# rvp-group/srrg2_proslam

Hardware: AMD Instinct MI355X
Metric: tracked frames/sec on KITTI-00 stereo (1241x376, ~2k kp); SE(3) vs ref (higher is better)
Workload: dtype u64 popcount (Hamming) + f32 (projection, Jacobians, 6x6 normal equations)

## Files before the change

srrg2_proslam_amd/csrc/align.hip:

```cpp
#include "prs_device.h"
#include "prs_host.h"
#include "prs_se3.h"

#include <math.h>
#include <string.h>

#include <type_traits>
#include <vector>

namespace prs {

constexpr int kAlignThreads = 256;
constexpr int kTerms        = 29;
constexpr uint32_t kNoneU32 = 0xffffffffu;
constexpr float kFltMax     = 3.402823466e+38f;

typedef unsigned int au32x4 __attribute__((ext_vector_type(4)));

struct AlignShared {
  float X[16];
  float A[16];
  float Sinv[16];
  float T[16];
  float Tprev[16];
// ... 1694 lines not shown
#pragma unroll
      for (int i = 0; i < 6; ++i) {
        b[i] = sh.b[i];
      }
      if (g.b.prior) {
        const float* pr = g.b.prior + (size_t) frame * 42;
#pragma unroll
        for (int i = 0; i < 36; ++i) {
          H[i] += pr[i];
        }
#pragma unroll
        for (int i = 0; i < 6; ++i) {
          b[i] += pr[36 + i];
        }
      }
#pragma unroll
      for (int i = 0; i < 16; ++i) {
        X[i] = sh.X[i];
      }
      if (g.a.enable_motion_prior) {
        add_motion_prior(g.a, g.prior_mean ? g.prior_mean + (size_t) frame * 16 : nullptr, X, H, b);
      }
      float dx6[6];
      const bool step_ok = gn_step(H, b, g.a.damping, X, g.a.damping_form == PRS_DAMPING_IDENTITY, dx6);
      const float dn2 = ((((dx6[0] * dx6[0] + dx6[1] * dx6[1]) + dx6[2] * dx6[2]) + dx6[3] * dx6[3]) + dx6[4] * dx6[4]) + dx6[5] * dx6[5];
      const bool small_step = g.a.step_norm_exit > 0.0f && step_ok && dn2 < g.a.step_norm_exit * g.a.step_norm_exit;
      uint32_t changed_bits = 0;
#pragma unroll
      for (int i = 0; i < 16; ++i) {
        changed_bits |= __float_as_uint(X[i]) ^ __float_as_uint(sh.X[i]);
        sh.X[i] = X[i];
      }
      float a16[16];
      pose_to_camera(g.a, sh.Sinv, X, a16);
#pragma unroll
      for (int i = 0; i < 16; ++i) {
        sh.A[i] = a16[i];
      }
      sh.decision = ((g.a.stop_at_fixed_point && changed_bits == 0u && (sh.converged || inlier_run)) || (small_step && (sh.converged || inlier_run))) ? 1 : 0;
    }
    __syncthreads();
    ALIGN_ACC(acc_solve);
    if (sh.decision) {
      if (!inlier_run && inlier_run_length(g.a) > 0) {
        it_align = g.a.max_iterations - 1;
        continue;
      }
      ++it_align;
      break;
    }
  }

  if (!split_search) {
    __syncthreads();
  }
  if (g.mode == PRS_MODE_ALIGN && !split_search && g.a.keep_only_inlier_correspondences && sh.have_cls && !sh.error) {
    const int nc = sh.n_corr;
    int base     = 0;
    for (int c0 = 0; c0 < nc; c0 += T) {
      const int c     = c0 + tid;
      const bool keep = c < nc && clsbuf[c] == 0;
      prs_corr cr;
      if (keep) {
        cr = gcorr[c];
      }
      const unsigned long long bal = __ballot(keep);
      if (lane == 0) {
        sh.wave_tot[wave] = __popcll(bal);
      }
      __syncthreads();
      int pos = base + __popcll(bal & ((1ull << lane) - 1ull));
      for (int w = 0; w < T / 64; ++w) {
        pos += w < wave ? sh.wave_tot[w] : 0;
        base += sh.wave_tot[w];
      }
      if (keep) {
        gcorr[pos] = cr;
      }
      __syncthreads();
    }
    if (tid == 0) {
      sh.n_corr = base;
    }
    __syncthreads();
  }

  if (split_search && lattice && !db_built && binds_disparity() && sh.error != PRS_ERR_CAPACITY) {
    bind_disparity();
  }

  if (!split_search) {
    __syncthreads();
  }
  if (tid < 16) {
    if (!split_search) {
      g.b.X[(size_t) frame * 16 + tid] = sh.X[tid];
    }
    gstate->local_map_in_sensor[tid]          = sh.T[tid];
    gstate->local_map_in_sensor_previous[tid] = sh.Tprev[tid];
  }
  for (int i = tid; i < 36; i += T) {
    gres->H[i] = sh.H[i];
  }
  if (tid < 6) {
    gres->b[tid] = sh.b[tid];
  }
  if (tid == 0) {
    gstate->search_radius_pixels = sh.radius;
    gstate->current_iteration    = sh.it;
    gstate->descriptor_distance  = sh.dd;
    gstate->database_leaf_range  = sh.kd_range;
    gstate->has_converged        = sh.converged;
    gstate->config_changed       = sh.config_changed;
    gstate->num_recomputes       = sh.num_recomputes;
    gstate->reserved             = (gstate->reserved & ~1) | sh.no_prune;
    g.b.n_corr[frame]            = sh.n_corr;
    gres->chi_inliers            = sh.chi_in;
    gres->chi_total              = sh.chi_tot;
    gres->mean_disparity         = sh.mean_disp;
    gres->num_inliers            = sh.n_inl;
    gres->num_outliers           = sh.n_out;
    gres->num_invalid            = sh.n_inv;
    gres->num_correspondences    = sh.n_corr;
    gres->status                 = sh.n_inl >= g.a.min_num_inliers ? 1 : 0;
    gres->iterations             = g.mode == PRS_MODE_ALIGN ? (ran_inlier_phase ? max_it : g.a.max_iterations) : 1;
    gres->iterations_executed    = executed;
    gres->warnings               = sh.error ? sh.error : sh.flags;
    if (split_search) {
      ctl->flags |= sh.flags;
      ctl->need_search = 0;
      gres->warnings   = sh.error ? sh.error : ctl->flags;
      if constexpr (kReuse) {
        ctl->q_tag = sh.q_tag & 0xffff;
      }
    }
    if (g.stamps) {
      unsigned long long* st = g.stamps + (size_t) frame * 16;
      st[0] = 0;
      for (int i = 0; i < 9; ++i) {
        st[i + 1] = st[i] + sh.stamp_acc[i];
      }
    }
  }
}

constexpr int kGnThreads = 128;
constexpr int kGnSlots   = 8;

struct GnShared {
  float X[16], T[16], Tprev[16];
  float H[36], b[6];
  float chi_in, chi_tot;
  float fcnt[3];
  float pad0;
  float A[16];
  float Sinv[16];
  float wsum[32];
  unsigned long long it;
  int converged, need_search, n_inl, n_out, n_inv, stop, flags;
  int pose_ok;
  int wave_tot[4];
};
static_assert(offsetof(GnShared, b) == offsetof(GnShared, H) + 36 * sizeof(float) && offsetof(GnShared, chi_in) == offsetof(GnShared, b) + 6 * sizeof(float) &&
                offsetof(GnShared, chi_tot) == offsetof(GnShared, chi_in) + sizeof(float) && offsetof(GnShared, fcnt) == offsetof(GnShared, chi_tot) + sizeof(float),
              "the summed slots are written through GnShared::H");

__device__ __forceinline__ bool gn_advance(const prs_aligner_params& a, const int extra, int& it_align, bool fixed_point, const int n_inl) {
  const bool was_inlier_run = it_align >= a.max_iterations;
  ++it_align;
  if (fixed_point && !was_inlier_run && extra > 0) {
    it_align    = a.max_iterations;
    fixed_point = false;
  }
  if (fixed_point) {
    return true;
  }
  if (it_align == a.max_iterations && extra > 0) {
    return n_inl < a.min_num_inliers;
  }
  return it_align >= a.max_iterations + extra;
}

template <bool SHIPPED_FORMS = false, int PLAIN = 0>
__device__ __forceinline__ void gn_solve_wave(const AlignArgs& g, GnShared& sh, const int frame, const int nc, const int stid, const bool inlier_run) {
  const int lane = stid;
  if (sh.pose_ok) {
    const int rrow = lane < 6 ? lane : 5;
    const int blk  = rrow >= 3 ? 1 : 0;
    const int ci   = rrow - 3 * blk;
    const float* Yb = &sh.H[18 * blk];
    const float Ri0 = sh.A[ci], Ri1 = sh.A[4 + ci], Ri2 = sh.A[8 + ci];
    float o[6];
#pragma unroll
    for (int cb = 0; cb < 2; ++cb) {
      float v[3];
#pragma unroll
      for (int c = 0; c < 3; ++c) {
        v[c] = fmaf(Ri2, Yb[12 + 3 * cb + c], fmaf(Ri1, Yb[6 + 3 * cb + c], Ri0 * Yb[3 * cb + c]));
      }
#pragma unroll
      for (int j = 0; j < 3; ++j) {
        o[3 * cb + j] = fmaf(v[2], sh.A[8 + j], fmaf(v[1], sh.A[4 + j], v[0] * sh.A[j]));
      }
    }
    const float bb = fmaf(Ri2, sh.b[3 * blk + 2], fmaf(Ri1, sh.b[3 * blk + 1], Ri0 * sh.b[3 * blk]));
    __builtin_amdgcn_fence(__ATOMIC_RELEASE, "wavefront");
    __builtin_amdgcn_wave_barrier();
    __builtin_amdgcn_fence(__ATOMIC_ACQUIRE, "wavefront");
    if (lane < 6) {
      float2* hw = reinterpret_cast<float2*>(&sh.H[6 * rrow]);
      hw[0]      = make_float2(o[0], o[1]);
      hw[1]      = make_float2(o[2], o[3]);
      hw[2]      = make_float2(o[4], o[5]);
      sh.b[rrow] = bb;
    }
    __builtin_amdgcn_fence(__ATOMIC_RELEASE, "wavefront");
    __builtin_amdgcn_wave_barrier();
    __builtin_amdgcn_fence(__ATOMIC_ACQUIRE, "wavefront");
  }
  if (stid == 0) {
    const int cc = (int) sh.fcnt[0];
    sh.n_inl     = cc & ((int) kClsOutUnit - 1);
    sh.n_out     = cc / (int) kClsOutUnit;
    sh.n_inv     = nc - sh.n_inl - sh.n_out;
  }
  {
    const int prow  = lane < 3 ? lane : 2;
    const float4 xr = *reinterpret_cast<const float4*>(&sh.X[4 * prow]);
    float H[36], b[6];
#pragma unroll
    for (int i = 0; i < 36; ++i) {
      H[i] = sh.H[i];
    }
#pragma unroll
    for (int i = 0; i < 6; ++i) {
      b[i] = sh.b[i];
    }
    if (PLAIN == 0 && g.b.prior) {
      const float* pr = g.b.prior + (size_t) frame * 42;
#pragma unroll
      for (int i = 0; i < 36; ++i) {
        H[i] += pr[i];
      }
#pragma unroll
      for (int i = 0; i < 6; ++i) {
        b[i] += pr[36 + i];
      }
    }
    if (PLAIN == 2 || (PLAIN == 0 && g.a.enable_motion_prior)) {
      float X[16];
#pragma unroll
      for (int i = 0; i < 16; ++i) {
        X[i] = sh.X[i];
      }
      add_motion_prior(g.a, g.prior_mean ? g.prior_mean + (size_t) frame * 16 : nullptr, X, H, b);
    }
    auto bcast = [](const float v, const int l) -> float { return __int_as_float(__builtin_amdgcn_readlane(__float_as_int(v), l)); };
    float dx[6];
    const bool ok = ldlt_solve6(H, b, g.a.damping, dx, !SHIPPED_FORMS && g.a.damping_form == PRS_DAMPING_IDENTITY);
    bool small_step = false;
    if (g.a.step_norm_exit > 0.0f) {
      const float n2 = ((((dx[0] * dx[0] + dx[1] * dx[1]) + dx[2] * dx[2]) + dx[3] * dx[3]) + dx[4] * dx[4]) + dx[5] * dx[5];
      small_step     = ok && n2 < g.a.step_norm_exit * g.a.step_norm_exit;
    }
    float D[16];
    tnq2t(dx, D);
    float4 xn;
    xn.x = (xr.x * D[0] + xr.y * D[4]) + xr.z * D[8];
    xn.y = (xr.x * D[1] + xr.y * D[5]) + xr.z * D[9];
    xn.z = (xr.x * D[2] + xr.y * D[6]) + xr.z * D[10];
    xn.w = ((xr.x * D[3] + xr.y * D[7]) + xr.z * D[11]) + xr.w;
    xn.x = ok ? xn.x : xr.x;
    xn.y = ok ? xn.y : xr.y;
    xn.z = ok ? xn.z : xr.z;
    xn.w = ok ? xn.w : xr.w;
    const uint32_t changed = (__float_as_uint(xn.x) ^ __float_as_uint(xr.x)) | (__float_as_uint(xn.y) ^ __float_as_uint(xr.y)) |
                             (__float_as_uint(xn.z) ^ __float_as_uint(xr.z)) | (__float_as_uint(xn.w) ^ __float_as_uint(xr.w));
    const bool any_changed = (__ballot(changed != 0u) & 7ull) != 0ull;
    float4 an = xn;
    if (PLAIN == 0 && g.a.with_sensor) {
      const float4 sr = *reinterpret_cast<const float4*>(&sh.Sinv[4 * prow]);
      const float4 x0 = {bcast(xn.x, 0), bcast(xn.y, 0), bcast(xn.z, 0), bcast(xn.w, 0)};
      const float4 x1 = {bcast(xn.x, 1), bcast(xn.y, 1), bcast(xn.z, 1), bcast(xn.w, 1)};
      const float4 x2 = {bcast(xn.x, 2), bcast(xn.y, 2), bcast(xn.z, 2), bcast(xn.w, 2)};
      an.x = (sr.x * x0.x + sr.y * x1.x) + sr.z * x2.x;
      an.y = (sr.x * x0.y + sr.y * x1.y) + sr.z * x2.y;
      an.z = (sr.x * x0.z + sr.y * x1.z) + sr.z * x2.z;
      an.w = ((sr.x * x0.w + sr.y * x1.w) + sr.z * x2.w) + sr.w;
    }
    const float rs = (an.x + an.y) + (an.z + an.w);
    const float fs = (bcast(rs, 0) + bcast(rs, 1)) + bcast(rs, 2);
    if (lane < 3) {
      *reinterpret_cast<float4*>(&sh.X[4 * lane]) = xn;
      *reinterpret_cast<float4*>(&sh.A[4 * lane]) = an;
    }
    if (stid == 0) {
      sh.stop    = ((g.a.stop_at_fixed_point && !any_changed && (sh.converged || inlier_run)) || (small_step && (sh.converged || inlier_run))) ? 1 : 0;
      sh.pose_ok = (fs - fs) == 0.0f ? 1 : 0;
    }
  }
}

__device__ __forceinline__ void gn_finder_bookkeeping(const AlignArgs& g, GnShared& sh, const int stid, const int nc, const int it_align, const int extra,
                                                      const bool fixed_point) {
    int next        = it_align;
    const bool over = gn_advance(g.a, extra, next, fixed_point, sh.n_inl);
    if (!over && next < g.a.max_iterations) {
      if (stid < 16) {
        sh.T[stid] = sh.A[stid];
      }
      if (!sh.converged) {
        const unsigned long long k  = g.f.number_of_solver_iterations_per_projection;
        const unsigned long long it = sh.it;
        if (k == 0 || it % k == 0 || it == 1) {
          if (stid == 0) {
            sh.need_search = 1;
          }
        } else {
          if (stid < 16) {
            sh.Tprev[stid] = sh.A[stid];
          }
          if (stid == 0) {
            sh.it = it + 1;
            if (nc == 0) {
              sh.flags |= PRS_WARN_NO_MATCHES;
            }
          }
        }
      } else if (stid == 0 && nc == 0) {
        sh.flags |= PRS_WARN_NO_MATCHES;
      }
    }
}

constexpr int kGnLdsSlots = 4;
constexpr size_t gn_lds_bytes(const int lds_slots) {
  return ((sizeof(GnShared) + 15) / 16) * 16 + (size_t) (lds_slots * 128 + 64) * 2 * sizeof(float4);
}
template <int SLOTS, int DIM, bool KEEP_CLS, int LDS_SLOTS = kGnLdsSlots, int WAVES = 4, int PLAIN = 0>
__global__ __launch_bounds__(128, WAVES) void gn_kernel(const AlignArgs g) {
  constexpr int THREADS = 128;
  constexpr int kGnLdsSlots = LDS_SLOTS;
  constexpr int kGnLdsRows  = LDS_SLOTS * 128 + 64;
  extern __shared__ __attribute__((aligned(16))) unsigned char smem[];
  const int tid   = threadIdx.x;
  const int lane  = tid & 63;
  const int wave  = tid >> 6;
  const int frame = blockIdx.x;
  const int solver = frame & 1;
  const int stid   = tid - 64 * solver;
  FrameCtl* ctl    = g.ctl + frame;
  constexpr int LS_IDX = (SLOTS < LDS_SLOTS ? SLOTS : LDS_SLOTS) + 1;
  const size_t fbase                    = (size_t) frame * (size_t) g.b.fixed_stride;
  const prs_corr* __restrict__ gcorr_in = g.b.corr + fbase;
  int fi[LS_IDX], mi[LS_IDX];
#pragma unroll
  for (int k = 0; k < LS_IDX; ++k) {
    const int c  = k * 128 + tid;
    const int cc = c < g.b.fixed_stride ? c : 0;
    fi[k]        = gcorr_in[cc].fixed_idx;
    mi[k]        = gcorr_in[cc].moving_idx;
  }
  if (ctl->done || ctl->need_search) {
    return;
  }
  GnShared& sh             = *reinterpret_cast<GnShared*>(smem);
  prs_pcf_state* gstate    = g.b.state + frame;
  prs_align_result* gres   = g.b.result + frame;
  const float4* gops       = g.ops + (size_t) frame * (size_t) g.max_fixed * 2;
  const int nc             = g.b.n_corr[frame];
  const float mean_dsp     = gres->mean_disparity;

  if (tid < 16) {
    sh.X[tid]     = g.b.X[(size_t) frame * 16 + tid];
    sh.T[tid]     = gstate->local_map_in_sensor[tid];
    sh.Tprev[tid] = gstate->local_map_in_sensor_previous[tid];
  }
  if (tid == 0) {
    sh.it          = gstate->current_iteration;
    sh.converged   = gstate->has_converged;
    sh.need_search = 0;
    sh.flags       = 0;
    sh.n_inl       = ctl->n_inl;
    sh.n_out       = ctl->n_out;
    sh.n_inv       = ctl->n_inv;
    sh.chi_in      = gres->chi_inliers;
    sh.chi_tot     = gres->chi_total;
    sh.stop        = 0;
    const float* gx = g.b.X + (size_t) frame * 16;
    float x[16], a16[16], si[16];
#pragma unroll
    for (int i = 0; i < 16; ++i) {
      x[i] = gx[i];
    }
    se3_inverse(g.a.sensor_in_robot, si);
    pose_to_camera(g.a, si, x, a16);
#pragma unroll
    for (int i = 0; i < 16; ++i) {
      sh.Sinv[i] = si[i];
      sh.A[i]    = a16[i];
    }
    const PoseRegs x0 = {a16[0], a16[1], a16[2], a16[3], a16[4], a16[5], a16[6], a16[7], a16[8], a16[9], a16[10], a16[11]};
    sh.pose_ok        = pose_is_finite(x0) ? 1 : 0;
  }
  for (int i = tid; i < 36; i += THREADS) {
    sh.H[i] = gres->H[i];
  }
  if (tid < 6) {
    sh.b[tid] = gres->b[tid];
  }
  constexpr int LS = SLOTS < kGnLdsSlots ? SLOTS : kGnLdsSlots;
  float4* lz = reinterpret_cast<float4*>(smem + ((sizeof(GnShared) + 15) / 16) * 16);
  constexpr int LROWS = SLOTS <= kGnLdsSlots ? SLOTS * THREADS : kGnLdsRows;
  float4* lp = lz + LROWS;
  const float4* __restrict__ gfix = reinterpret_cast<const float4*>(g.b.fixed) + fbase;
  const float4* __restrict__ gmov = reinterpret_cast<const float4*>(g.b.moving) + (size_t) frame * (size_t) g.b.moving_stride;
  if (nc > 0) {
    static_assert(LS_IDX == LS + 1, "index pairs of the parked rows");
    float4 zr[LS + 1], pr[LS + 1];
#pragma unroll
    for (int k = 0; k < LS + 1; ++k) {
      const bool live = k * THREADS + tid < nc;
      zr[k]           = gfix[live ? fi[k] : 0];
      pr[k]           = gmov[live ? mi[k] : 0];
    }
#pragma unroll
    for (int k = 0; k < LS + 1; ++k) {
      const int c = k * THREADS + tid;
      if (k * THREADS < nc && c < LROWS) {
        float4 z = c < nc ? zr[k] : make_float4(0.f, 0.f, 0.f, 0.f);
        z.w      = parked_translation_weight(g.a, z, mean_dsp, DIM != 0 ? 0 : g.a.translation_weight_form);
        lz[c]    = z;
        lp[c]    = c < nc ? pr[k] : make_float4(0.f, 0.f, 1.f, 1.f);
      }
    }
  }
  if (SLOTS > kGnLdsSlots) {
    float4* wops = g.ops + (size_t) frame * (size_t) g.max_fixed * 2;
#pragma unroll
    for (int k = LS; k < SLOTS; ++k) {
      const int c = k * THREADS + tid;
      if (c >= LROWS && c < nc) {
        const int fi    = gcorr_in[c].fixed_idx, mi = gcorr_in[c].moving_idx;
        float4 z        = gfix[fi];
        z.w             = parked_translation_weight(g.a, z, mean_dsp, DIM != 0 ? 0 : g.a.translation_weight_form);
        wops[2 * c]     = z;
        wops[2 * c + 1] = gmov[mi];
      }
    }
  }
  const int my_slot = (lane >> 1) & 31;
  const int sum_dst = gn_slot_destination(my_slot, (lane & 1) != 0);
  __syncthreads();

  int it_align = ctl->it_align;
  int executed = ctl->executed;
  bool done    = false;
  const int extra = PLAIN != 0 ? 0 : inlier_run_length(g.a);
  uint32_t cls_bits = 0;
  bool have_cls     = false;


  while (true) {
    ++executed;
    if (nc < g.a.min_num_correspondences) {
      if (tid == 0) {
        sh.n_inl = sh.n_out = sh.n_inv = 0;
        sh.chi_in = sh.chi_tot = 0.0f;
        sh.stop = (g.a.stop_at_fixed_point && (sh.converged || it_align >= g.a.max_iterations)) ? 1 : 0;
      }
      for (int i = tid; i < 36; i += THREADS) {
        sh.H[i] = 0.0f;
      }
      if (tid < 6) {
        sh.b[tid] = 0.0f;
      }
      have_cls = false;
      __syncthreads();
      if (wave == solver) {
        gn_finder_bookkeeping(g, sh, stid, nc, it_align, extra, sh.stop != 0);
      }
      __syncthreads();
    } else {
      const bool inlier_run = PLAIN == 0 && it_align >= g.a.max_iterations;
      have_cls              = true;
      cls_bits              = 0;
      const PoseRegs pose = {sh.A[0], sh.A[1], sh.A[2], sh.A[3], sh.A[4], sh.A[5], sh.A[6], sh.A[7], sh.A[8], sh.A[9], sh.A[10], sh.A[11]};
      const bool pose_ok  = __builtin_amdgcn_readfirstlane(sh.pose_ok) != 0;
      f2 acc[kPairs];
#pragma unroll
      for (int i = 0; i < kPairs; ++i) {
        acc[i] = f2{0.0f, 0.0f};
      }
      float code = 0.0f;
      if (pose_ok) {
#pragma unroll
        for (int k = 0; k < SLOTS; ++k) {
          const int c0 = k * THREADS;
          if (k == 0 || c0 + 64 * wave < nc) {
            const int c = c0 + tid;
            float4 z, p;
            if (k < LS || (k == LS && c0 + 64 * wave < LROWS)) {
              z = lz[c];
              p = lp[c];
            } else {
              const int cs = cold_copy(c);
              z   = c < nc ? gops[2 * cs] : make_float4(0.f, 0.f, 0.f, 1.f);
              p   = c < nc ? gops[2 * cs + 1] : make_float4(0.f, 0.f, 1.f, 1.f);
            }
            int cls;
            factor_accumulate<DIM, true>(g.a, pose, z, p, mean_dsp, c < nc, acc, code, cls, inlier_run);
            if (KEEP_CLS) {
              cls_bits |= (uint32_t) (cls & 3) << (2 * k);
            }
          }
        }
      } else if (KEEP_CLS) {
#pragma unroll
        for (int k = 0; k < SLOTS; ++k) {
          if (k * THREADS + tid < nc) {
            cls_bits |= 2u << (2 * k);
          }
        }
      }
      acc[kSlotCls >> 1].x = code;
      float tot = wave_sum_slots(acc, lane);
      if (wave != solver) {
        sh.wsum[my_slot] = tot;
      }
      __syncthreads();
      if (wave == solver) {
        tot = tot + sh.wsum[my_slot];
        tot = tot + 0.0f;
        (&sh.H[0])[sum_dst] = tot;
        __builtin_amdgcn_fence(__ATOMIC_RELEASE, "wavefront");
        __builtin_amdgcn_wave_barrier();
        __builtin_amdgcn_fence(__ATOMIC_ACQUIRE, "wavefront");
        gn_solve_wave<DIM != 0, PLAIN>(g, sh, frame, nc, stid, inlier_run);
        __builtin_amdgcn_fence(__ATOMIC_RELEASE, "wavefront");
        __builtin_amdgcn_wave_barrier();
        __builtin_amdgcn_fence(__ATOMIC_ACQUIRE, "wavefront");
        gn_finder_bookkeeping(g, sh, stid, nc, it_align, extra, sh.stop != 0);
      }
      __syncthreads();
    }
    if (gn_advance(g.a, extra, it_align, sh.stop != 0, sh.n_inl)) {
      done = true;
      break;
    }
    if (it_align < g.a.max_iterations && sh.need_search) {
      break;
    }
  }

  int nc_out = nc;
  __syncthreads();
  if (KEEP_CLS && done && g.a.keep_only_inlier_correspondences && have_cls) {
    prs_corr* __restrict__ gcorr = g.b.corr + (size_t) frame * (size_t) g.b.fixed_stride;
    int base                     = 0;
#pragma unroll
    for (int k = 0; k < SLOTS; ++k) {
      const int c0 = k * THREADS;
      if (c0 < nc) {
        const int c     = c0 + tid;
        const bool keep = c < nc && ((cls_bits >> (2 * k)) & 3u) == 0u;
        prs_corr cr;
        if (keep) {
          cr = gcorr[c];
        }
        const unsigned long long bal = __ballot(keep);
        if (lane == 0) {
          sh.wave_tot[wave] = __popcll(bal);
        }
        __syncthreads();
        int pos = base + __popcll(bal & ((1ull << lane) - 1ull));
#pragma unroll
        for (int w = 0; w < THREADS / 64; ++w) {
          pos += w < wave ? sh.wave_tot[w] : 0;
          base += sh.wave_tot[w];
        }
        if (keep) {
          gcorr[pos] = cr;
        }
        __syncthreads();
      }
    }
    nc_out = base;
  }

  __syncthreads();
  if (tid < 16) {
    g.b.X[(size_t) frame * 16 + tid]           = sh.X[tid];
    gstate->local_map_in_sensor[tid]          = sh.T[tid];
    gstate->local_map_in_sensor_previous[tid] = sh.Tprev[tid];
  }
  for (int i = tid; i < 36; i += THREADS) {
    const int r = i / 6, c = i - 6 * r;
    gres->H[i]  = sh.H[r >= c ? i : 6 * c + r];
  }
  if (tid < 6) {
    gres->b[tid] = sh.b[tid];
  }
  if (tid == 0) {
    gstate->current_iteration = sh.it;
    gres->chi_inliers         = sh.chi_in;
    gres->chi_total           = sh.chi_tot;
    gres->num_inliers         = sh.n_inl;
    gres->num_outliers        = sh.n_out;
    gres->num_invalid         = sh.n_inv;
    gres->num_correspondences = nc_out;
    if (nc_out != nc) {
      g.b.n_corr[frame] = nc_out;
    }
    gres->status              = sh.n_inl >= g.a.min_num_inliers ? 1 : 0;
    gres->iterations          = it_align > g.a.max_iterations ? g.a.max_iterations + extra : g.a.max_iterations;
    gres->iterations_executed = executed;
    ctl->flags |= sh.flags;
    gres->warnings   = ctl->flags;
    ctl->it_align    = it_align;
    ctl->executed    = executed;
    ctl->n_inl       = sh.n_inl;
    ctl->n_out       = sh.n_out;
    ctl->n_inv       = sh.n_inv;
    ctl->need_search = done ? 0 : 1;
    ctl->done        = done ? 1 : 0;
    if (!done) {
      atomicAdd(g.pending, 1);
    }
  }
}

__global__ void split_init_kernel(FrameCtl* ctl, prs_align_result* res, int* pending, int batch) {
  const int i = blockIdx.x * blockDim.x + threadIdx.x;
  if (i < batch) {
    FrameCtl c;
    c.it_align    = 0;
    c.need_search = 1;
    c.done        = 0;
    c.executed    = 0;
    c.flags       = 0;
    c.n_inl = c.n_out = c.n_inv = 0;
    c.db_ready                  = 0;
    c.q_tag = c.q_hits = c.q_misses = 0;
    ctl[i]                      = c;
    prs_align_result r;
    for (int k = 0; k < 36; ++k) {
      r.H[k] = 0.0f;
    }
    for (int k = 0; k < 6; ++k) {
      r.b[k] = 0.0f;
    }
    r.chi_inliers = r.chi_total = r.mean_disparity = 0.0f;
    r.num_inliers = r.num_outliers = r.num_invalid = r.num_correspondences = 0;
    r.status = r.iterations = r.iterations_executed = r.warnings = 0;
    res[i]                                                        = r;
  }
  if (i == 0) {
    *pending = 0;
  }
}

__global__ void gn_step_kernel(const float* H, const float* b, float damping, int identity_damping, float* X, int* ok) {
  float h[36], bb[6], x[16];
  for (int i = 0; i < 36; ++i) {
    h[i] = H[i];
  }
  for (int i = 0; i < 6; ++i) {
    bb[i] = b[i];
  }
  for (int i = 0; i < 16; ++i) {
    x[i] = X[i];
  }
  const bool r = gn_step(h, bb, damping, x, identity_damping != 0);
  for (int i = 0; i < 16; ++i) {
    X[i] = x[i];
  }
  *ok = r ? 1 : 0;
}

static inline uint32_t align_up16(uint32_t v) {
  return (v + 15u) / 16u * 16u;
}

struct SplitJob {
  bool active = false;
  bool last   = false;
  void* own[6]        = {nullptr, nullptr, nullptr, nullptr, nullptr, nullptr};
  size_t own_bytes[6] = {0, 0, 0, 0, 0, 0};
  hipStream_t stream  = nullptr;
  hipStream_t capture_stream = nullptr;
  ~SplitJob() {
    for (void* p : own) {
      if (p) {
        (void) hipFree(p);
      }
    }
  }
  void* buffer(hipStream_t s, int i, size_t bytes) {
    if (bytes <= own_bytes[i]) {
      return own[i];
    }
    if (own[i]) {
      (void) hipStreamSynchronize(s);
      (void) hipFree(own[i]);
      own[i]       = nullptr;
      own_bytes[i] = 0;
    }
    const size_t want = bytes + bytes / 4 + 4096;
    if (hipMalloc(&own[i], want) != hipSuccess) {
      own[i] = nullptr;
      return nullptr;
    }
    own_bytes[i] = want;
    return own[i];
  }
  AlignArgs g, gs;
  void (*search)(AlignArgs) = nullptr;
  void (*gn)(AlignArgs)     = nullptr;
  size_t lds_search = 0, lds_gn = 0;
  int total = 0, limit = 0;
  int enqueued = 0;
  int ev_used = 0;
  int rounds_timed = 0;
  bool stamps = false;
};
static int split_rounds(prs_context* ctx, SplitJob* job, int rounds);

#define AK(...) PRS_VARIANT("prs::", align_kernel, AlignArgs, __VA_ARGS__)
#define GN(...) PRS_VARIANT("prs::", gn_kernel, AlignArgs, __VA_ARGS__)
static const Variant<AlignArgs> kAlignVariants[] = {
    AK(256, false, -1, 4),
    AK(512, true, 2, 8), AK(512, true, 2, 4), AK(512, true, 1, 8), AK(512, true, 1, 4), AK(512, true, 3, 8), AK(512, true, 3, 4), AK(512, true, 0, 4),
    GN(4, 4, false, 4, 1, 1), GN(4, 4, false, 4, 1, 0), GN(8, 4, false, 4, 1, 1), GN(8, 4, false, 4, 1, 0),
    GN(4, 4, false, 4, 4, 2), GN(4, 4, false, 4, 4, 0), GN(4, 4, false, 4, 4, 1), GN(4, 3, true, 4, 4, 0), GN(4, 0, true, 4, 4, 0),
    GN(8, 4, false, 3, 5, 2), GN(8, 4, false, 3, 5, 0), GN(8, 4, false, 3, 5, 1), GN(8, 3, true, 4, 4, 0), GN(8, 0, true, 4, 4, 0),
};
#undef AK
#undef GN
static_assert(kAlignThreads == 256 && kSearchThreads == 512 && kGnLdsSlots == 4 && PRS_SEARCH_KDTREE == 0 && PRS_SEARCH_SQUARE == 1 && PRS_SEARCH_CIRCLE == 2 &&
                PRS_SEARCH_RHOMBUS == 3 && PRS_FACTOR_DEPTH == 3 && PRS_FACTOR_STEREO == 4,
              "kAlignVariants spells these as literals");

const char* align_kernel_name(int index) {
  return index >= 0 && index < (int) (sizeof(kAlignVariants) / sizeof(kAlignVariants[0])) ? kAlignVariants[index].name : nullptr;
}

struct AlignPlan : Plan {
  AlignArgs g = {}, gs = {};
  bool split = false, stamps_split = false;
  bool reuse = false;
  bool lone = false, five = false, fast = false, plain = false, mprior = false, depth = false;
};

static AlignPlan align_plan(const prs_pcf_params& finder, const prs_aligner_params& aligner, const prs_align_batch& batch, int mode, const DispatchEnv& env) {
  AlignPlan p;
  if (mode < PRS_MODE_ALIGN || mode > PRS_MODE_LINEARIZE) {
    p.refuse(PRS_ERR_UNSUPPORTED, "prs_align_batch_run: unknown mode");
    return p;
  }
  if (batch.batch <= 0) {
    return p;
  }
  if (batch.fixed_stride <= 0 || batch.fixed_stride > 32767 || batch.moving_stride <= 0 || batch.moving_stride > 65535) {
    p.refuse(PRS_ERR_UNSUPPORTED, "prs_align_batch_run: fixed_stride must be in [1,32767], moving_stride in [1,65535]");
    return p;
  }
  if (finder.projector.canvas_rows <= 0 || finder.projector.canvas_rows > 8192 || finder.projector.canvas_cols <= 0 ||
      finder.projector.canvas_cols > 32767) {
    p.refuse(PRS_ERR_UNSUPPORTED, "prs_align_batch_run: projector canvas must be within 32767 x 8192");
    return p;
  }
  if (finder.maximum_search_radius_pixels > 16383 || finder.search_type < PRS_SEARCH_KDTREE || finder.search_type > PRS_SEARCH_RHOMBUS) {
    p.refuse(PRS_ERR_UNSUPPORTED, "prs_align_batch_run: search radius > 16383 px or unknown search type");
    return p;
  }
  if (aligner.factor_type != PRS_FACTOR_MONO && aligner.factor_type != PRS_FACTOR_DEPTH && aligner.factor_type != PRS_FACTOR_STEREO) {
    p.refuse(PRS_ERR_UNSUPPORTED, "prs_align_batch_run: factor_type must be 2, 3 or 4");
    return p;
  }
  if ((aligner.kernel_weight_form != PRS_KERNEL_WEIGHT_INV_CHI && aligner.kernel_weight_form != PRS_KERNEL_WEIGHT_TAU_OVER_CHI) ||
      (aligner.damping_form != PRS_DAMPING_DIAG && aligner.damping_form != PRS_DAMPING_IDENTITY) ||
      (aligner.translation_weight_form != PRS_TRANSLATION_WEIGHT_OFFSET && aligner.translation_weight_form != PRS_TRANSLATION_WEIGHT_CLAMP)) {
    p.refuse(PRS_ERR_UNSUPPORTED, "prs_align_batch_run: unknown kernel_weight_form / damping_form / translation_weight_form");
// ... 97 lines not shown
  p.add(find_variant(kAlignVariants, {kSearchThreads, 1, finder.search_type, gs.surv_slots}), batch.batch, 1, kSearchThreads, lds_search);
  p.reuse = !env.no_search_reuse && !kdtree && gs.surv_slots == 4 && ncx <= 256 && ncy <= 256 && max_fixed < 2048;
  p.fast = aligner.factor_type == PRS_FACTOR_STEREO && !aligner.keep_only_inlier_correspondences && aligner.kernel_weight_form == PRS_KERNEL_WEIGHT_INV_CHI &&
           aligner.damping_form == PRS_DAMPING_DIAG && aligner.translation_weight_form == PRS_TRANSLATION_WEIGHT_OFFSET;
  p.lone = p.fast && batch.batch <= 2 * env.cus && !env.no_lone_gn;
  p.five = p.fast && !p.lone && max_fixed > 4 * 128;
  const bool lean = !batch.prior && !aligner.with_sensor && !aligner.enable_inlier_only_runs;
  p.plain  = lean && !aligner.enable_motion_prior;
  p.mprior = lean && aligner.enable_motion_prior;
  p.depth = aligner.factor_type == PRS_FACTOR_DEPTH && aligner.kernel_weight_form == PRS_KERNEL_WEIGHT_INV_CHI && aligner.damping_form == PRS_DAMPING_DIAG;
  const int slots = max_fixed <= 4 * 128 ? 4 : 8, lds_slots = p.five ? 3 : kGnLdsSlots;
  const int gn    = p.fast ? find_variant(kAlignVariants, {slots, PRS_FACTOR_STEREO, 0, lds_slots, p.lone ? 1 : (p.five ? 5 : 4),
                                                           p.plain ? 1 : (p.mprior && !p.lone ? 2 : 0)})
                           : find_variant(kAlignVariants, {slots, p.depth ? PRS_FACTOR_DEPTH : 0, 1, kGnLdsSlots, 4, 0});
  p.add(gn, batch.batch, 1, kGnThreads, gn_lds_bytes(lds_slots));
  return p;
}

int align_batch_launch(prs_context* ctx, const prs_pcf_params* finder, const prs_aligner_params* aligner, const prs_align_batch* batch, int mode, int rounds) {
  if (ctx->align_job && static_cast<SplitJob*>(ctx->align_job)->active) {
    return ctx_fail(ctx, PRS_ERR_UNSUPPORTED, "prs_align_batch_*: the previous batch of this context has not been finished (prs_align_batch_finish)");
  }
  if (!finder || !aligner || !batch || !batch->fixed || !batch->fixed_desc || !batch->n_fixed || !batch->moving ||
      !batch->moving_desc || !batch->n_moving || !batch->state || !batch->X || !batch->corr || !batch->n_corr || !batch->result) {
    return ctx_fail(ctx, PRS_ERR_NULL, "prs_align_batch_run: fixed, moving, correspondences, state or result not set");
  }
  const AlignPlan plan = align_plan(*finder, *aligner, *batch, mode, dispatch_env(ctx));
  if (plan.status != PRS_OK) {
    return ctx_fail(ctx, plan.status, plan.message);
  }
  if (plan.n_launches == 0) {
    return PRS_OK;
  }
  unsigned long long* stamps = ctx_stamps(ctx, (size_t) batch->batch * 16 * sizeof(unsigned long long));
  auto with_inputs = [&](AlignArgs a) {
    a.f          = *finder;
    a.a          = *aligner;
    a.b          = *batch;
    a.no_prefilter = ctx->no_prefilter ? 1 : 0;
    a.narrow_prefilter_limit = ctx->prefilter_96_limit;
    a.prior_mean = batch->prior_mean;
    a.stamps     = stamps;
    return a;
  };
  AlignArgs g        = with_inputs(plan.g);
  hipStream_t stream = ctx_stream(ctx);
  hipError_t e;
  if (!plan.split) {
    const Plan::Launch& l = plan.launch[0];
    auto kernel = kAlignVariants[l.kernel].fn;
    e           = hipFuncSetAttribute(reinterpret_cast<const void*>(kernel), hipFuncAttributeMaxDynamicSharedMemorySize, (int) l.lds);
    if (e != hipSuccess) {
      return ctx_fail_hip(ctx, e, "prs_align_batch_run attribute");
    }
    hipLaunchKernelGGL(kernel, dim3(l.grid_x), dim3(l.block), l.lds, stream, g);
    if (ctx->align_job) {
      static_cast<SplitJob*>(ctx->align_job)->last = false;
    }
    e = hipGetLastError();
    if (e != hipSuccess) {
      return ctx_fail_hip(ctx, e, "prs_align_batch_run launch");
    }
    if (g.stamps) {
      ctx_report_stamps(ctx, batch->batch, 10, "align (fused, 256 threads): finder | linearize + in-wave reduction | cross-wave sum | GN solve || of finder: lattice build | projection+search | staging (keys, fixed rows -> LDS) | filter | commit");
    }
    return PRS_OK;
  }
  const Plan::Launch &ls = plan.launch[0], &lg = plan.launch[1];
  SplitJob* job = static_cast<SplitJob*>(ctx->align_job);
  if (!job) {
    job                 = new SplitJob();
    ctx->align_job      = job;
    ctx->align_job_free = [](void* p) { delete static_cast<SplitJob*>(p); };
  }
  const int max_fixed    = g.max_fixed;
  const size_t ops_bytes = (size_t) batch->batch * (size_t) max_fixed * 2 * sizeof(float4);
  const size_t ctl_bytes = (size_t) batch->batch * sizeof(FrameCtl) + 256;
  unsigned char* small   = static_cast<unsigned char*>(job->buffer(stream, 0, ctl_bytes));
  g.ops                  = static_cast<float4*>(job->buffer(stream, 1, ops_bytes));
  if (!small || !g.ops) {
    return ctx_fail(ctx, PRS_ERR_HIP, "prs_align_batch_run: split-pipeline scratch allocation failed");
  }
  g.pending = reinterpret_cast<int*>(small);
  g.ctl     = reinterpret_cast<FrameCtl*>(small + 256);
  AlignArgs gs = with_inputs(plan.gs);
  gs.ops       = g.ops;
  gs.pending   = g.pending;
  gs.ctl       = g.ctl;
  gs.dbcache   = static_cast<unsigned char*>(job->buffer(stream, 2, (size_t) batch->batch * gs.db_blob));
  if (!gs.dbcache) {
    return ctx_fail(ctx, PRS_ERR_HIP, "prs_align_batch_run: lattice cache allocation failed");
  }
  if (finder->search_type != PRS_SEARCH_KDTREE) {
    gs.rowcache = static_cast<au32x4*>(job->buffer(stream, 3, (size_t) batch->batch * (size_t) max_fixed * 2 * sizeof(au32x4)));
    if (!gs.rowcache) {
      return ctx_fail(ctx, PRS_ERR_HIP, "prs_align_batch_run: descriptor row cache allocation failed");
    }
  }
  if (plan.reuse) {
    const size_t queries = (size_t) batch->batch * (size_t) batch->moving_stride;
    gs.qcache            = static_cast<au32x4*>(job->buffer(stream, 4, queries * sizeof(au32x4)));
    gs.missq             = gs.qcache ? static_cast<uint16_t*>(job->buffer(stream, 5, queries * sizeof(uint16_t))) : nullptr;
    if (!gs.missq) {
      (void) hipGetLastError();
      gs.qcache = nullptr;
    }
  }
  e = hipFuncSetAttribute(reinterpret_cast<const void*>(kAlignVariants[ls.kernel].fn), hipFuncAttributeMaxDynamicSharedMemorySize, (int) ls.lds);
  if (e != hipSuccess) {
    return ctx_fail_hip(ctx, e, "prs_align_batch_run attribute");
  }
  hipLaunchKernelGGL(split_init_kernel, dim3((batch->batch + 255) / 256), dim3(256), 0, stream, g.ctl, batch->result, g.pending, batch->batch);
  job->active      = true;
  job->stream      = stream;
  job->capture_stream = stream;
  job->g           = g;
  job->gs          = gs;
  job->search      = kAlignVariants[ls.kernel].fn;
  job->gn          = kAlignVariants[lg.kernel].fn;
  job->last        = true;
  job->lds_search  = ls.lds;
  job->lds_gn      = lg.lds;
  job->total       = 0;
  job->limit       = 2 * (aligner->max_iterations + inlier_run_length(*aligner)) + 8;
  job->ev_used     = 0;
  job->rounds_timed = 0;
  job->stamps      = plan.stamps_split && stamps;
  job->enqueued    = rounds > 0 ? rounds : 5;
  return split_rounds(ctx, job, job->enqueued);
}

static int split_rounds(prs_context* ctx, SplitJob* job, int rounds) {
  hipStream_t stream = job->stream;
  auto tick = [&]() {
    if (ctx->timing && job->ev_used < 3 * 64) {
      if (!ctx->timing_ev[job->ev_used]) {
        (void) hipEventCreate(&ctx->timing_ev[job->ev_used]);
      }
      (void) hipEventRecord(ctx->timing_ev[job->ev_used], stream);
      ++job->ev_used;
    }
  };
  const int batch = job->g.b.batch;
  for (int r = 0; r < rounds; ++r) {
    (void) hipMemsetAsync(job->g.pending, 0, sizeof(int), stream);
    tick();
    hipLaunchKernelGGL(job->search, dim3(batch), dim3(kSearchThreads), job->lds_search, stream, job->gs);
    tick();
    if (job->stamps) {
      ctx_report_stamps(ctx, batch, 10, "search launch (split): - | query-cache pass | - | - || lattice build | projection+search (behind a cache pass: the scan of its queue) | staging (keys, fixed rows -> LDS) | filter | commit");
    }
    hipLaunchKernelGGL(job->gn, dim3(batch), dim3(kGnThreads), job->lds_gn, stream, job->g);
    tick();
    ++job->total;
  }
  const hipError_t e = hipGetLastError();
  if (e != hipSuccess) {
    job->active = false;
    return ctx_fail_hip(ctx, e, "prs_align_batch_run split launch");
  }
  return PRS_OK;
}

int align_batch_finish(prs_context* ctx) {
  SplitJob* job = static_cast<SplitJob*>(ctx->align_job);
  if (!job || !job->active) {
    return PRS_OK;
  }
  hipStream_t stream = job->stream;
  auto collect = [&]() {
    for (int i = 0; i + 2 < job->ev_used; i += 3) {
      float a = 0.f, b = 0.f;
      if (hipEventElapsedTime(&a, ctx->timing_ev[i], ctx->timing_ev[i + 1]) == hipSuccess &&
          hipEventElapsedTime(&b, ctx->timing_ev[i + 1], ctx->timing_ev[i + 2]) == hipSuccess) {
        ctx->t_search_ms += a;
        ctx->t_gn_ms += b;
        ++ctx->n_search;
        ++ctx->n_gn;
        const int round = job->rounds_timed < 15 ? job->rounds_timed : 15;
        ctx->t_search_round[round] += a;
        ctx->t_gn_round[round] += b;
      }
      ++job->rounds_timed;
    }
    job->ev_used = 0;
  };
  for (;;) {
    int pending  = 0;
    hipError_t e = hipMemcpyAsync(&pending, job->g.pending, sizeof(int), hipMemcpyDeviceToHost, stream);
    if (e == hipSuccess) {
      e = hipStreamSynchronize(stream);
    }
    if (e != hipSuccess) {
      job->active = false;
      return ctx_fail_hip(ctx, e, "prs_align_batch_finish: completion check");
    }
    collect();
    if (pending == 0) {
      break;
    }
    if (job->total > job->limit) {
      job->active = false;
      return ctx_fail(ctx, PRS_ERR_HIP, "prs_align_batch_finish: split pipeline did not finish");
    }
    const int rc = split_rounds(ctx, job, 4);
    if (rc != PRS_OK) {
      return rc;
    }
  }
  job->active = false;
  if (ctx->timing) {
    ++ctx->n_batches_timed;
  }
  return PRS_OK;
}

int align_batch_rearm(prs_context* ctx, hipStream_t replay_stream) {
  SplitJob* job = static_cast<SplitJob*>(ctx->align_job);
  if (!job || !job->gn) {
    return ctx_fail(ctx, PRS_ERR_UNSUPPORTED, "prs_align_batch_rearm: no batch has been enqueued on this context");
  }
  if (job->active) {
    return ctx_fail(ctx, PRS_ERR_UNSUPPORTED, "prs_align_batch_rearm: the previous batch has not been finished");
  }
  job->stream       = replay_stream ? replay_stream : job->capture_stream;
  job->active       = true;
  job->total        = job->enqueued;
  job->ev_used      = 0;
  job->rounds_timed = 0;
  return PRS_OK;
}

int align_reuse_counts(prs_context* ctx, long long* hits, long long* misses) {
  *hits = *misses = 0;
  SplitJob* job = static_cast<SplitJob*>(ctx->align_job);
  if (!job || !job->gn || !job->last) {
    return PRS_OK;
  }
  if (job->active) {
    return ctx_fail(ctx, PRS_ERR_UNSUPPORTED, "prs_context_get_search_reuse: the batch has not been finished (prs_align_batch_finish)");
  }
  std::vector<FrameCtl> ctl((size_t) job->g.b.batch);
  hipError_t e = hipMemcpyAsync(ctl.data(), job->g.ctl, ctl.size() * sizeof(FrameCtl), hipMemcpyDeviceToHost, job->stream);
  if (e == hipSuccess) {
    e = hipStreamSynchronize(job->stream);
  }
  if (e != hipSuccess) {
    return ctx_fail_hip(ctx, e, "prs_context_get_search_reuse");
  }
  for (const FrameCtl& c : ctl) {
    *hits += c.q_hits;
    *misses += c.q_misses;
  }
  return PRS_OK;
}

bool align_job_active(const prs_context* ctx) {
  const SplitJob* job = static_cast<const SplitJob*>(ctx->align_job);
  return job && job->active;
}

__global__ __launch_bounds__(256) void recip_selftest_kernel(unsigned long long* counts) {
  const uint32_t stride = gridDim.x * blockDim.x;
  unsigned long long differ = 0, fast = 0;
  for (uint64_t i = (uint64_t) blockIdx.x * blockDim.x + threadIdx.x; i < (1ull << 32); i += stride) {
    const float x  = __uint_as_float((uint32_t) i);
    const float ax = __builtin_fabsf(x);
    const bool short_form = __ballot(!(ax >= 0x1p-126f && ax < 0x1p126f)) == 0ull;
    const uint32_t got = __float_as_uint(recip_exact(x)), want = __float_as_uint(1.0f / x);
    const bool both_nan = (got & 0x7fffffffu) > 0x7f800000u && (want & 0x7fffffffu) > 0x7f800000u;
    differ += (got != want && !both_nan) ? 1ull : 0ull;
    fast += short_form ? 1ull : 0ull;
  }
  if (differ) {
    atomicAdd(&counts[0], differ);
  }
  atomicAdd(&counts[1], fast);
}

int recip_selftest_launch(prs_context* ctx, unsigned long long* d_counts) {
  hipLaunchKernelGGL(recip_selftest_kernel, dim3(256 * 32), dim3(256), 0, ctx_stream(ctx), d_counts);
  hipError_t e = hipGetLastError();
  if (e != hipSuccess) {
    return ctx_fail_hip(ctx, e, "prs_selftest_reciprocal launch");
  }
  return PRS_OK;
}

int gn_step_launch(prs_context* ctx, const float* dH, const float* db, float damping, int damping_form, float* dX, int* dok) {
  hipLaunchKernelGGL(gn_step_kernel, dim3(1), dim3(1), 0, ctx_stream(ctx), dH, db, damping, damping_form == PRS_DAMPING_IDENTITY ? 1 : 0, dX, dok);
  hipError_t e = hipGetLastError();
  if (e != hipSuccess) {
    return ctx_fail_hip(ctx, e, "prs_gn_step launch");
  }
  return PRS_OK;
}

}

extern "C" int prs_align_plan(const prs_pcf_params* finder, const prs_aligner_params* aligner, const prs_align_batch* batch, int32_t mode,
                              const prs_dispatch_env* env, prs_dispatch_plan* out) {
  if (!finder || !aligner || !batch || !env || !out) {
    return PRS_ERR_NULL;
  }
  const prs::AlignPlan p = prs::align_plan(*finder, *aligner, *batch, mode, *env);
  prs::export_plan(p, prs::kAlignVariants, out);
// ... 10 lines not shown
```

Baseline: 1.949 million.

## Gather GN kernel header state with one per-lane load and readlane broadcasts

Replaces the scattered scalar reads of the frame control block, n_corr, result header, pose and state at gn_kernel entry with a single 32-bit load per lane. Each lane is mapped to one header word, the values are broadcast through readlane or stored straight into LDS, and the early-exit test uses the loaded words, so idle workgroups leave after one load. The spill rows beyond the LDS slots now reuse the already-fetched extra row and batch their index and row loads, and the PLAIN variant skips the pose-to-camera transform. It also adds optional clock64 stamps behind a compile flag, and it depends on strict struct-offset assumptions that are checked with static_asserts.

```diff
diff --git a/srrg2_proslam_amd/csrc/align.hip b/srrg2_proslam_amd/csrc/align.hip
--- a/srrg2_proslam_amd/csrc/align.hip
+++ b/srrg2_proslam_amd/csrc/align.hip
@@ -1870,7 +1870,7 @@
   float H[36], b[6];
   float chi_in, chi_tot;
   float fcnt[3];
-  float pad0;
+  int flags_in;
   float A[16];
   float Sinv[16];
   float wsum[32];
@@ -2055,6 +2055,11 @@
 constexpr size_t gn_lds_bytes(const int lds_slots) {
   return ((sizeof(GnShared) + 15) / 16) * 16 + (size_t) (lds_slots * 128 + 64) * 2 * sizeof(float4);
 }
+#ifdef PRS_GN_STAMPS
+#define GN_STAMP(i) do { if (g.stamps) { asm volatile("" ::: "memory"); gn_clk[i] = (unsigned long long) clock64(); asm volatile("" ::: "memory"); } } while (0)
+#else
+#define GN_STAMP(i) do { } while (0)
+#endif
 template <int SLOTS, int DIM, bool KEEP_CLS, int LDS_SLOTS = kGnLdsSlots, int WAVES = 4, int PLAIN = 0>
 __global__ __launch_bounds__(128, WAVES) void gn_kernel(const AlignArgs g) {
   constexpr int THREADS = 128;
@@ -2068,6 +2073,68 @@
   const int solver = frame & 1;
   const int stid   = tid - 64 * solver;
   FrameCtl* ctl    = g.ctl + frame;
+#ifdef PRS_GN_STAMPS
+  unsigned long long gn_clk[6] = {0, 0, 0, 0, 0, 0};
+#endif
+  GN_STAMP(0);
+  typedef uint32_t __attribute__((may_alias)) hword_t;
+  static_assert(sizeof(FrameCtl) == 48 && offsetof(FrameCtl, it_align) == 0 && offsetof(FrameCtl, need_search) == 4 && offsetof(FrameCtl, done) == 8 &&
+                  offsetof(FrameCtl, executed) == 12 && offsetof(FrameCtl, flags) == 16 && offsetof(FrameCtl, n_inl) == 20 && offsetof(FrameCtl, n_inv) == 28,
+                "lanes 0-11 of the header load are the control word");
+  static_assert(offsetof(prs_align_result, b) == offsetof(prs_align_result, H) + 36 * sizeof(float) &&
+                  offsetof(prs_align_result, chi_total) == offsetof(prs_align_result, chi_inliers) + sizeof(float) &&
+                  offsetof(prs_pcf_state, local_map_in_sensor_previous) == offsetof(prs_pcf_state, local_map_in_sensor) + 16 * sizeof(float) &&
+                  offsetof(GnShared, T) == offsetof(GnShared, X) + 16 * sizeof(float) && offsetof(GnShared, Tprev) == offsetof(GnShared, T) + 16 * sizeof(float) &&
+                  offsetof(GnShared, n_inv) == offsetof(GnShared, n_inl) + 2 * sizeof(int) && offsetof(GnShared, it) % 8 == 0,
+                "runs of header words that consecutive lanes load and store");
+  prs_pcf_state* gstate  = g.b.state + frame;
+  prs_align_result* gres = g.b.result + frame;
+  const hword_t* hsrc    = reinterpret_cast<const hword_t*>(ctl);
+  int hdst               = -1;
+  {
+    constexpr int kResH = offsetof(prs_align_result, H) / 4, kResChi = offsetof(prs_align_result, chi_inliers) / 4, kResMd = offsetof(prs_align_result, mean_disparity) / 4;
+    constexpr int kStT = offsetof(prs_pcf_state, local_map_in_sensor) / 4, kStIt = offsetof(prs_pcf_state, current_iteration) / 4, kStConv = offsetof(prs_pcf_state, has_converged) / 4;
+    constexpr int kShX = offsetof(GnShared, X), kShChi = offsetof(GnShared, chi_in), kShH = offsetof(GnShared, H), kShIt = offsetof(GnShared, it);
+    constexpr int kShConv = offsetof(GnShared, converged), kShInl = offsetof(GnShared, n_inl), kShFlags = offsetof(GnShared, flags_in);
+    const int l   = lane;
+    const bool w1 = wave != 0;
+    int rec = 0, word = l;
+    auto run = [&](const bool in, const int r, const int w, const int d) {
+      rec  = in ? r : rec;
+      word = in ? w : word;
+      hdst = in ? d : hdst;
+    };
+    run(l == 12, 1, 0, -1);
+    run(l == 13, 2, kResMd, -1);
+    run(!w1 && l >= 14 && l < 16, 2, kResChi + (l - 14), kShChi + 4 * (l - 14));
+    run(!w1 && l >= 16 && l < 32, 3, l - 16, kShX + 4 * (l - 16));
+    run(!w1 && l >= 32, 4, kStT + (l - 32), kShX + 4 * (l - 16));
+    run(w1 && l == 4, 0, l, kShFlags);
+    run(w1 && l >= 5 && l < 8, 0, l, kShInl + 4 * (l - 5));
+    run(w1 && l == 14, 4, kStConv, kShConv);
+    run(w1 && l >= 15 && l < 17, 4, kStIt + (l - 15), kShIt + 4 * (l - 15));
+    run(w1 && l >= 17 && l < 59, 2, kResH + (l - 17), kShH + 4 * (l - 17));
+    run(w1 && l >= 59, 0, 0, -1);
+    const hword_t* base = reinterpret_cast<const hword_t*>(ctl);
+    base                = rec == 1 ? reinterpret_cast<const hword_t*>(g.b.n_corr + frame) : base;
+    base                = rec == 2 ? reinterpret_cast<const hword_t*>(gres) : base;
+    base                = rec == 3 ? reinterpret_cast<const hword_t*>(g.b.X + (size_t) frame * 16) : base;
+    base                = rec == 4 ? reinterpret_cast<const hword_t*>(gstate) : base;
+    hsrc                = base + word;
+  }
+  const int hw = (int) *hsrc;
+  if (__builtin_amdgcn_readlane(hw, 2) | __builtin_amdgcn_readlane(hw, 1)) {
+#ifdef PRS_GN_STAMPS
+    if (g.stamps && tid == 0) {
+      for (int i = 0; i < 7; ++i) {
+        g.stamps[(size_t) frame * 16 + i] = 0;
+      }
+    }
+#endif
+    return;
+  }
+  GN_STAMP(1);
+  GN_STAMP(2);
   constexpr int LS_IDX = (SLOTS < LDS_SLOTS ? SLOTS : LDS_SLOTS) + 1;
   const size_t fbase                    = (size_t) frame * (size_t) g.b.fixed_stride;
   const prs_corr* __restrict__ gcorr_in = g.b.corr + fbase;
@@ -2079,53 +2146,47 @@
     fi[k]        = gcorr_in[cc].fixed_idx;
     mi[k]        = gcorr_in[cc].moving_idx;
   }
-  if (ctl->done || ctl->need_search) {
-    return;
-  }
-  GnShared& sh             = *reinterpret_cast<GnShared*>(smem);
-  prs_pcf_state* gstate    = g.b.state + frame;
-  prs_align_result* gres   = g.b.result + frame;
-  const float4* gops       = g.ops + (size_t) frame * (size_t) g.max_fixed * 2;
-  const int nc             = g.b.n_corr[frame];
-  const float mean_dsp     = gres->mean_disparity;
-
-  if (tid < 16) {
-    sh.X[tid]     = g.b.X[(size_t) frame * 16 + tid];
-    sh.T[tid]     = gstate->local_map_in_sensor[tid];
-    sh.Tprev[tid] = gstate->local_map_in_sensor_previous[tid];
-  }
-  if (tid == 0) {
-    sh.it          = gstate->current_iteration;
-    sh.converged   = gstate->has_converged;
-    sh.need_search = 0;
-    sh.flags       = 0;
-    sh.n_inl       = ctl->n_inl;
-    sh.n_out       = ctl->n_out;
-    sh.n_inv       = ctl->n_inv;
-    sh.chi_in      = gres->chi_inliers;
-    sh.chi_tot     = gres->chi_total;
-    sh.stop        = 0;
-    const float* gx = g.b.X + (size_t) frame * 16;
-    float x[16], a16[16], si[16];
+  GnShared& sh         = *reinterpret_cast<GnShared*>(smem);
+  const float4* gops   = g.ops + (size_t) frame * (size_t) g.max_fixed * 2;
+  const int nc         = __builtin_amdgcn_readlane(hw, 12);
+  const float mean_dsp = __int_as_float(__builtin_amdgcn_readlane(hw, 13));
+  const int it_align0  = __builtin_amdgcn_readlane(hw, 0);
+  const int executed0  = __builtin_amdgcn_readlane(hw, 3);
+  if (hdst >= 0) {
+    *reinterpret_cast<hword_t*>(smem + hdst) = (hword_t) hw;
+  }
+  if (wave == 0) {
+    float x[16];
 #pragma unroll
     for (int i = 0; i < 16; ++i) {
-      x[i] = gx[i];
-    }
-    se3_inverse(g.a.sensor_in_robot, si);
-    pose_to_camera(g.a, si, x, a16);
-#pragma unroll
-    for (int i = 0; i < 16; ++i) {
-      sh.Sinv[i] = si[i];
-      sh.A[i]    = a16[i];
-    }
-    const PoseRegs x0 = {a16[0], a16[1], a16[2], a16[3], a16[4], a16[5], a16[6], a16[7], a16[8], a16[9], a16[10], a16[11]};
-    sh.pose_ok        = pose_is_finite(x0) ? 1 : 0;
-  }
-  for (int i = tid; i < 36; i += THREADS) {
-    sh.H[i] = gres->H[i];
-  }
-  if (tid < 6) {
-    sh.b[tid] = gres->b[tid];
+      x[i] = __int_as_float(__builtin_amdgcn_readlane(hw, 16 + i));
+    }
+    if (tid == 0) {
+      sh.need_search = 0;
+      sh.flags       = 0;
+      sh.stop        = 0;
+      float a16[16];
+      if (PLAIN != 0) {
+#pragma unroll
+        for (int i = 0; i < 16; ++i) {
+          a16[i] = x[i];
+        }
+      } else {
+        float si[16];
+        se3_inverse(g.a.sensor_in_robot, si);
+        pose_to_camera(g.a, si, x, a16);
+#pragma unroll
+        for (int i = 0; i < 16; ++i) {
+          sh.Sinv[i] = si[i];
+        }
+      }
+#pragma unroll
+      for (int i = 0; i < 16; ++i) {
+        sh.A[i] = a16[i];
+      }
+      const PoseRegs x0 = {a16[0], a16[1], a16[2], a16[3], a16[4], a16[5], a16[6], a16[7], a16[8], a16[9], a16[10], a16[11]};
+      sh.pose_ok        = pose_is_finite(x0) ? 1 : 0;
+    }
   }
   constexpr int LS = SLOTS < kGnLdsSlots ? SLOTS : kGnLdsSlots;
   float4* lz = reinterpret_cast<float4*>(smem + ((sizeof(GnShared) + 15) / 16) * 16);
@@ -2142,6 +2203,7 @@
       zr[k]           = gfix[live ? fi[k] : 0];
       pr[k]           = gmov[live ? mi[k] : 0];
     }
+    GN_STAMP(2);
 #pragma unroll
     for (int k = 0; k < LS + 1; ++k) {
       const int c = k * THREADS + tid;
@@ -2152,27 +2214,60 @@
         lp[c]    = c < nc ? pr[k] : make_float4(0.f, 0.f, 1.f, 1.f);
       }
     }
-  }
-  if (SLOTS > kGnLdsSlots) {
-    float4* wops = g.ops + (size_t) frame * (size_t) g.max_fixed * 2;
-#pragma unroll
-    for (int k = LS; k < SLOTS; ++k) {
-      const int c = k * THREADS + tid;
-      if (c >= LROWS && c < nc) {
-        const int fi    = gcorr_in[c].fixed_idx, mi = gcorr_in[c].moving_idx;
-        float4 z        = gfix[fi];
-        z.w             = parked_translation_weight(g.a, z, mean_dsp, DIM != 0 ? 0 : g.a.translation_weight_form);
-        wops[2 * c]     = z;
-        wops[2 * c + 1] = gmov[mi];
-      }
-    }
+    if (SLOTS > kGnLdsSlots) {
+      float4* wops = g.ops + (size_t) frame * (size_t) g.max_fixed * 2;
+      {
+        const int c = LS * THREADS + tid;
+        if (c >= LROWS && c < nc) {
+          float4 z        = zr[LS];
+          z.w             = parked_translation_weight(g.a, z, mean_dsp, DIM != 0 ? 0 : g.a.translation_weight_form);
+          wops[2 * c]     = z;
+          wops[2 * c + 1] = pr[LS];
+        }
+      }
+      constexpr int NS = SLOTS - LS - 1;
+      if (NS > 0 && nc > (LS + 1) * THREADS) {
+        int fs[NS > 0 ? NS : 1], ms[NS > 0 ? NS : 1];
+#pragma unroll
+        for (int k = 0; k < NS; ++k) {
+          const int c  = (LS + 1 + k) * THREADS + tid;
+          const int cc = c < nc ? c : 0;
+          fs[k]        = gcorr_in[cc].fixed_idx;
+          ms[k]        = gcorr_in[cc].moving_idx;
+        }
+        typedef float row_t __attribute__((ext_vector_type(4)));
+        row_t zs[NS > 0 ? NS : 1], ps[NS > 0 ? NS : 1];
+#pragma unroll
+        for (int k = 0; k < NS; ++k) {
+          const bool live = (LS + 1 + k) * THREADS + tid < nc;
+          zs[k]           = *reinterpret_cast<const row_t*>(gfix + (live ? fs[k] : 0));
+          ps[k]           = *reinterpret_cast<const row_t*>(gmov + (live ? ms[k] : 0));
+        }
+#pragma unroll
+        for (int k = 0; k < NS; ++k) {
+          const int c = (LS + 1 + k) * THREADS + tid;
+          if (c < nc) {
+            float4 z = make_float4(zs[k].x, zs[k].y, zs[k].z, 0.0f);
+            z.w      = parked_translation_weight(g.a, z, mean_dsp, DIM != 0 ? 0 : g.a.translation_weight_form);
+            *reinterpret_cast<row_t*>(wops + 2 * c)     = row_t{z.x, z.y, z.z, z.w};
+            *reinterpret_cast<row_t*>(wops + 2 * c + 1) = ps[k];
+          }
+        }
+      }
+    }
+  } else {
+    float4 z = make_float4(0.f, 0.f, 0.f, 0.f);
+    z.w      = parked_translation_weight(g.a, z, mean_dsp, DIM != 0 ? 0 : g.a.translation_weight_form);
+    lz[tid]  = z;
+    lp[tid]  = make_float4(0.f, 0.f, 1.f, 1.f);
   }
   const int my_slot = (lane >> 1) & 31;
   const int sum_dst = gn_slot_destination(my_slot, (lane & 1) != 0);
   __syncthreads();
-
-  int it_align = ctl->it_align;
-  int executed = ctl->executed;
+  GN_STAMP(3);
+
+  int it_align = it_align0;
+  int executed = executed0;
   bool done    = false;
   const int extra = PLAIN != 0 ? 0 : inlier_run_length(g.a);
   uint32_t cls_bits = 0;
@@ -2273,6 +2368,7 @@
 
   int nc_out = nc;
   __syncthreads();
+  GN_STAMP(4);
   if (KEEP_CLS && done && g.a.keep_only_inlier_correspondences && have_cls) {
     prs_corr* __restrict__ gcorr = g.b.corr + (size_t) frame * (size_t) g.b.fixed_stride;
     int base                     = 0;
@@ -2333,8 +2429,9 @@
     gres->status              = sh.n_inl >= g.a.min_num_inliers ? 1 : 0;
     gres->iterations          = it_align > g.a.max_iterations ? g.a.max_iterations + extra : g.a.max_iterations;
     gres->iterations_executed = executed;
-    ctl->flags |= sh.flags;
-    gres->warnings   = ctl->flags;
+    const int flags  = sh.flags_in | sh.flags;
+    ctl->flags       = flags;
+    gres->warnings   = flags;
     ctl->it_align    = it_align;
     ctl->executed    = executed;
     ctl->n_inl       = sh.n_inl;
@@ -2345,8 +2442,19 @@
     if (!done) {
       atomicAdd(g.pending, 1);
     }
-  }
-}
+#ifdef PRS_GN_STAMPS
+    GN_STAMP(5);
+    if (g.stamps) {
+      unsigned long long* st = g.stamps + (size_t) frame * 16;
+      for (int i = 0; i < 6; ++i) {
+        st[i] = gn_clk[i] - gn_clk[0];
+      }
+      st[6] = st[5] + 1000;
+    }
+#endif
+  }
+}
+#undef GN_STAMP
 
 __global__ void split_init_kernel(FrameCtl* ctl, prs_align_result* res, int* pending, int batch) {
   const int i = blockIdx.x * blockDim.x + threadIdx.x;
@@ -2750,6 +2858,11 @@
     }
     hipLaunchKernelGGL(job->gn, dim3(batch), dim3(kGnThreads), job->lds_gn, stream, job->g);
     tick();
+#ifdef PRS_GN_STAMPS
+    if (job->stamps) {
+      ctx_report_stamps(ctx, batch, 7, "Gauss-Newton launch (split), mean over ALL workgroups (idle ones count zero): entry to control decision | decision to gather issued | gather to first barrier | iterations | write-back | 1000 x share of active workgroups");
+    }
+#endif
     ++job->total;
   }
   const hipError_t e = hipGetLastError();
```

Result: no change. 1.943 million (-0.3%).
